# brucechin/OctopusZK

Hardware: AMD Instinct MI355X
Metric: BN254 G1 VariableBaseMSM Mscalar-mul/s at 2^20 (higher is better)
Workload: dtype u32; 1 GPU; VariableBaseMSM BN254 G1 2^20 random scalars/bases per GPU, bit-exact vs the serial CPU path (BASELINE.json configs[1]); n_per_gpu=1048576, window_bits=16, windows=8, glv=True, prepared_bases=False, msms_in_flight=3, schedule=pipeline3, parallelism=index-range shard x1, RCCL all-gather of 192-B partials + HIP point sum

## Files before the change

### octopuszk_amd/csrc/knobs.h

```cpp
#pragma once
#include <stdlib.h>
#include <string.h>

#include <atomic>
#include <mutex>

namespace ozk {

constexpr int KNOB_COMPUTED = -0x7fffffff;
constexpr int KNOB_STRING = KNOB_COMPUTED + 1;

#define OZK_KNOBS(X)                                                                                                     \
                                                   \
  X(MSM_GLV, "OZK_MSM_GLV", 1, "0: plain 256-bit windows instead of the GLV split (var MSM up to 2^23 pairs, fixed base)") \
  X(MSM_SIGNED, "OZK_MSM_SIGNED", 1, "0: unsigned window digits in the GLV form")                                        \
  X(MSM_C, "OZK_MSM_C", KNOB_COMPUTED, "window bits, 1..16 (default: the cost model's choice)")                          \
  X(MSM_L1, "OZK_MSM_L1", KNOB_COMPUTED, "sorted entries per level-1 lane (default: from the bucket size; 0 as unset)")   \
  X(MSM_L1_WHOLE, "OZK_MSM_L1_WHOLE", 1, "G1 level 1 by whole buckets on lane groups: 0 never, 1 on every plan that can take it (unset: where it pays)") \
  X(MSM_L1_ROUNDS, "OZK_MSM_L1_ROUNDS", 2, "most rounds of resident workgroups level 1 is rounded up to; 0: no rounding") \
  X(MSM_TAIL_MODE, "OZK_MSM_TAIL_MODE", -1, "0 / 1: force the latency / throughput shape of the window sums")            \
  X(MSM_TAIL_RC, "OZK_MSM_TAIL_RC", -1, "1: G1 throughput window sums by bucket rows and columns wherever the buffers take them (0 / unset: the serial levels)") \
  X(MSM_SMALL_SORT, "OZK_MSM_SMALL_SORT", 1, "0: small MSMs take the two-level sort too")                                \
  X(MSM_S_LAT, "OZK_MSM_S_LAT", KNOB_COMPUTED, "buckets per lane in a latency tail's fused first level (default: 8 G1, 4 G2)") \
  X(MSM_FIN_MAX, "OZK_MSM_FIN_MAX", 4, "elements per window left to the final one-wave kernel, 1..16")                   \
                                                                                                    \
  X(HOST_SLICES, "OZK_HOST_SLICES", 8, "most slices a host-buffer MSM is cut into; 1: no slicing")                       \
  X(HOST_SLICE_MIN_LOG, "OZK_HOST_SLICE_MIN_LOG", 18, "log2 of the smallest slice")                                      \
  X(SHARD, "OZK_SHARD", 0, "1: the JNI entries shard large calls over the visible devices")                              \
  X(SHARD_MIN_N, "OZK_SHARD_MIN_N", 1 << 21, "smallest call OZK_SHARD=1 shards")                                         \
  X(SHARD_COUNT, "OZK_SHARD_COUNT", 0, "shards of such a call; 0: one per device")                                       \
  X(SHARD_RCCL, "OZK_SHARD_RCCL", 1, "0: the partials of a sharded call go through the host, not RCCL")                  \
  X(COPY_HELPERS, "OZK_COPY_HELPERS", 3, "threads staging host buffers beside the caller, 0..11 (first use only)")       \
  X(HOST_TRACE, "OZK_HOST_TRACE", 0, "1: per-call host timings on stderr; 2: with absolute timestamps")                  \
                                                                                     \
  X(FB_WS, "OZK_FB_WS", KNOB_COMPUTED, "window bits of a GLV fixed-base table (default: cost model, at most the caller's)") \
  X(FB_AFFINE, "OZK_FB_AFFINE", 1, "0: Jacobian gather-add instead of affine table records")                             \
  X(FB_TABLE_CACHE, "OZK_FB_TABLE_CACHE", 1, "0: window tables are built per call")                                      \
  X(FB_TABLE_CACHE_MB, "OZK_FB_TABLE_CACHE_MB", 1024, "MiB of cached window tables per device")                          \
  X(FB_TABLE_CACHE_SECOND_USE, "OZK_FB_TABLE_CACHE_SECOND_USE", 1, "0: a table is cached on its first use")              \
  X(FB_HOST_RANGES, "OZK_FB_HOST_RANGES", 4, "ranges a host fixed-base call downloads its results in")                   \
  X(MM_WS, "OZK_MM_WS", KNOB_COMPUTED, "window bits of the shared-base batched MSM (default: from n)")                   \
                                                                                             \
  X(FFT_MAXK, "OZK_FFT_MAXK", 8, "most butterfly stages per pass, 3..10")                                                \
  X(FFT_PLAN, "OZK_FFT_PLAN", 1, "0: stages spread evenly over the passes")                                              \
  X(FFT_KS, "OZK_FFT_KS", KNOB_STRING, "explicit stages per pass, e.g. \"8,6,8\" (must sum to log2 n)")                  \
  X(FFT_TW_PYRAMID, "OZK_FFT_TW_PYRAMID", 1, "0: twiddles from the flat table")                                          \
  X(FFT_PLAN_CACHE, "OZK_FFT_PLAN_CACHE", 1, "0: twiddle tables are built per call")                                     \
  X(FFT_PLAN_CACHE_MB, "OZK_FFT_PLAN_CACHE_MB", 4096, "MiB of cached twiddle tables per device")                         \
  X(QAP_FOLD_SCALE, "OZK_QAP_FOLD_SCALE", 1, "0: the witness map scales in a pass of its own")                           \
  X(BACE_LDS_SLOTS, "OZK_BACE_LDS_SLOTS", 16, "circuit slots kept in LDS, 0..28")

enum Knob {
#define X(id, env, dflt, doc) K_##id,
  OZK_KNOBS(X)
#undef X
  K_COUNT
};
struct KnobInfo {
  const char* env;
  int dflt;
  const char* doc;
};
inline constexpr KnobInfo KNOBS[K_COUNT] = {
#define X(id, env, dflt, doc) {env, dflt, doc},
    OZK_KNOBS(X)
#undef X
};

struct KnobSnapshot {
  bool has[K_COUNT];
  int val[K_COUNT];
// ... 39 lines not shown
```

### octopuszk_amd/csrc/l1_whole.h

```cpp
#pragma once
#include <stdint.h>

#if !defined(OZK_HD)
#if defined(__HIPCC__)
#include <hip/hip_runtime.h>
#define OZK_HD __host__ __device__ __forceinline__
#else
#define OZK_HD inline
#endif
#endif

namespace ozk {

constexpr int WHOLE_G = 2;
constexpr int WHOLE_LANE_MAX = 255;
constexpr int WHOLE_NB_MAX = 128;

struct WholeGeom {
  int W;
  int NH;
  int nb;
  int g_top;
};
OZK_HD int whole_nbins(const WholeGeom& g) { return g.W * g.NH; }
constexpr uint32_t WHOLE_NO_ITEM = 0xffffffffu;
OZK_HD int whole_pad4(int x) { return (x + 3) & ~3; }
OZK_HD int whole_lanes_per_rank(const WholeGeom& g) {
  return whole_pad4(WHOLE_G * g.NH * (g.W - 1)) + whole_pad4(g.g_top * g.NH);
}
OZK_HD long long whole_lanes(const WholeGeom& g) { return (long long)g.nb * whole_lanes_per_rank(g); }
OZK_HD int whole_group(const WholeGeom& g, int bin) { return bin / g.NH == g.W - 1 ? g.g_top : WHOLE_G; }
OZK_HD uint32_t whole_limit(int G) { return (uint32_t)(G * WHOLE_LANE_MAX); }

OZK_HD uint32_t whole_rank(const uint32_t* cnt, int nb, int i) {
  const uint32_t c = cnt[i];
  uint32_t r = 0;
  for (int j = 0; j < nb; j++) r += (cnt[j] > c) || (cnt[j] == c && j < i);
  return r;
}
OZK_HD uint32_t whole_item_index(uint32_t rank, uint32_t bin, uint32_t nbins) { return rank * nbins + bin; }

OZK_HD void whole_lane_map(const WholeGeom& geo, uint32_t t, uint32_t* item, uint32_t* g, uint32_t* G) {
  const uint32_t per_rank = (uint32_t)whole_lanes_per_rank(geo);
  const uint32_t rank = t / per_rank, q = t - rank * per_rank;
  const uint32_t ordinary = (uint32_t)(WHOLE_G * geo.NH * (geo.W - 1));
  const uint32_t ordinary_pad = (uint32_t)whole_pad4((int)ordinary);
  uint32_t bin;
  bool pad;
  if (q < ordinary_pad) {
    bin = q / WHOLE_G;
    *g = q % WHOLE_G;
    *G = WHOLE_G;
    pad = q >= ordinary;
  } else {
    const uint32_t q2 = q - ordinary_pad;
    bin = (uint32_t)(geo.NH * (geo.W - 1)) + q2 / (uint32_t)geo.g_top;
    *g = q2 % (uint32_t)geo.g_top;
    *G = (uint32_t)geo.g_top;
    pad = q2 >= (uint32_t)(geo.g_top * geo.NH);
  }
  *item = pad ? WHOLE_NO_ITEM : whole_item_index(rank, bin, (uint32_t)whole_nbins(geo));
}

OZK_HD void whole_part(uint32_t count, uint32_t g, uint32_t G, uint32_t* first, uint32_t* len) {
  const uint32_t a = (count * g + G - 1) / G, b = (count * (g + 1) + G - 1) / G;
  *first = a;
  *len = b - a;
}

}
```

### octopuszk_amd/csrc/msm_var.cuh

```cuda
#pragma once
#include "curve.cuh"
#include "glv.cuh"
#include "l1_whole.h"
#include "wsum_rc.h"

namespace ozk {

constexpr u32 BID_NONE = 0xffffffffu;

struct MsmPlan {
  int n_in;
  int glv;
  int n;
  int sd;
  int c;
  int cb;
  int W;
  int L1;
  int LK;
  int S;
  int lone;
  int small_sort;
  int S_lat;
  int fin_max;
  int tail_mode;
  int tail_rc;
  int l1_whole;
  int l1_gtop;
};

OZK_HD u32 scalar_digit(const u32 (&s)[8], int w, int c) {
  const int bit = w * c;
  const int wi = bit >> 5, sh = bit & 31;
  u32 v = s[wi] >> sh;
  if (sh + c > 32 && wi + 1 < 8) v |= s[wi + 1] << (32 - sh);
  return v & ((1u << c) - 1u);
}

OZK_HD bool digit_decode(u32 code, int sd, u32& b, u32& neg) {
  if (sd) {
    const u32 t = code - 1u;
    b = t >> 1;
    neg = t & 1u;
  } else {
    b = code;
    neg = 0;
  }
  return code != 0;
}
template <class Emit>
OZK_HD void signed_digit_codes(const u32 (&e)[8], int c, int W, bool neg, Emit emit) {
  const u32 half = 1u << (c - 1);
  const u32 thr = (c == 16 && neg) ? half - 1u : half;
  u32 cy = 0;
  for (int w = 0; w < W; w++) {
    const u32 d = scalar_digit(e, w, c) + cy;
    cy = d > thr;
    const u32 m = cy ? (1u << c) - d : d;
    emit(w, (uint16_t)(m ? (((m - 1u) << 1) | (cy ^ (u32)neg)) + 1u : 0u));
  }
}

constexpr u32 SIDX_NEG = 0x80000000u;

#if defined(__HIPCC__)


template <class CV>
__global__ void __launch_bounds__(256) k_convert_bases(const u32* __restrict__ wire,
                                                       u32* __restrict__ aff, int n, int glv,
                                                       const uint8_t* __restrict__ neg_flags) {
  using IO = CurveIO<CV>;
  using EA = typename CV::EA;
  using ET = ElemTraits<EA>;
  const int i = blockIdx.x * blockDim.x + threadIdx.x;
  if (i >= n) return;
  const u32* p = wire + (size_t)i * IO::WIRE_JAC_WORDS;
  u32* o = aff + (size_t)i * IO::AFF_WORDS;
  Aff<EA> q;
  if (ET::wire_is_zero(p + 2 * IO::CW)) {
    q.x = EA(el_zero(q.x));
// ... 1004 lines not shown
          for (int q = s + 1; q <= e; q += 2) acc = xyzz_add(acc, IO::load_xyzz(pts + (size_t)q * IO::REC_WORDS));
          IO::store_rec_xyzz(acc, buckets + (size_t)bx * IO::REC_WORDS);
        } else if (e > s) {
          const u32 j = atomicAdd(&item_cnt[0], 1u);
          item_s[0][j] = (u32)s;
          item_span[0][j] = (uint8_t)(e - s);
        } else {
          IO::store_rec_xyzz(IO::load_xyzz(pts + (size_t)s * IO::REC_WORDS), buckets + (size_t)bx * IO::REC_WORDS);
        }
      }
    }
    bid_out[x] = out;
    alive += (out != BID_NONE);
  }
  if (t == 0 && n_slots > 0) {
    bid_out[0] = bid_in[0];
    alive += (bid_in[0] != BID_NONE);
  }
  for (int o = 32; o > 0; o >>= 1) alive += __shfl_xor(alive, o);
  if ((threadIdx.x & 63) == 0 && alive) atomicAdd(remaining, alive);
#pragma unroll 1
  for (int r = 0; LIST && r < ROUNDS; r++) {
    block_sync();
    const u32 len = (u32)__builtin_amdgcn_readfirstlane((int)item_cnt[r]);
    if (len == 0) break;
    const int cur = r & 1;
#pragma unroll 1
    for (u32 i = threadIdx.x; i < len; i += RUNMERGE_BLOCK) {
      const u32 s = item_s[cur][i];
      const u32 span = item_span[cur][i];
      u32* bucket = buckets + (size_t)bid_in[s] * IO::REC_WORDS;
      const u32 off = 2u * (u32)r + 1u;
      const u32* sum = r == 0 ? pts + (size_t)s * IO::REC_WORDS : bucket;
      const Xyzz<CV> acc = xyzz_add(IO::load_xyzz(sum), IO::load_xyzz(pts + ((size_t)s + off) * IO::REC_WORDS));
      IO::store_rec_xyzz(acc, bucket);
      if (off + 2u <= span) {
        const u32 j = atomicAdd(&item_cnt[r + 1], 1u);
        item_s[cur ^ 1][j] = s;
        item_span[cur ^ 1][j] = (uint8_t)span;
      }
    }
  }
}

constexpr int ITEMS_BLOCK = WHOLE_NB_MAX;
__device__ __forceinline__ u32 items_block_sum(u32 v, u32* wsum) {
#pragma unroll
  for (int o = 32; o > 0; o >>= 1) v += __shfl_xor(v, o);
  if ((threadIdx.x & 63) == 0) wsum[threadIdx.x >> 6] = v;
  block_sync();
  return wsum[0] + wsum[1];
}
static __global__ void __launch_bounds__(ITEMS_BLOCK)
k_bin_sums(const u32* __restrict__ hist, WholeGeom geo, int cb, int lo_bits, u32* __restrict__ binsum) {
  static_assert(ITEMS_BLOCK == 128, "two waves");
  __shared__ u32 wsum[2];
  const int t = threadIdx.x, bin = blockIdx.x;
  const int w = bin / geo.NH, h = bin - w * geo.NH;
  const u32 bucket0 = ((u32)w << cb) | ((u32)h << lo_bits);
  const u32 sum = items_block_sum(t < geo.nb ? hist[bucket0 + t] : 0u, wsum);
  if (t == 0) binsum[bin] = sum;
}
static __global__ void __launch_bounds__(ITEMS_BLOCK)
k_bucket_items(const u32* __restrict__ hist, const u32* __restrict__ binsum, WholeGeom geo, int cb, int lo_bits,
               u32 big_thresh, uint4* __restrict__ items, u32* __restrict__ bad) {
  __shared__ u32 cnt[WHOLE_NB_MAX];
  __shared__ u32 wsum[2];
  const int t = threadIdx.x, bin = blockIdx.x;
  const int w = bin / geo.NH, h = bin - w * geo.NH;
  const u32 bucket0 = ((u32)w << cb) | ((u32)h << lo_bits);
  const u32 c = t < geo.nb ? hist[bucket0 + t] : 0u;
  cnt[t] = c;
  u32 before = 0;
  for (int j = t; j < bin; j += ITEMS_BLOCK) before += binsum[j];
  const u32 base = items_block_sum(before, wsum);
  if (t >= geo.nb) return;
  u32 excl = 0, sum = 0;
  for (int j = 0; j < geo.nb; j++) {
    const u32 cj = cnt[j];
    sum += cj;
    excl += j < t ? cj : 0u;
  }
  const u32 rank = whole_rank(cnt, geo.nb, t);
  items[whole_item_index(rank, (u32)bin, (u32)whole_nbins(geo))] = make_uint4(base + excl, c, bucket0 + (u32)t, 0u);
  if (c > whole_limit(whole_group(geo, bin)) || sum > big_thresh) *bad = 1u;
}

template <int CTRL, class CV>
__device__ __forceinline__ Xyzz<CV> xyzz_quad_swap(const Xyzz<CV>& a) {
  using IO = CurveIO<CV>;
  constexpr int RW = IO::RW;
  u32 w[4 * RW];
  ElemTraits<typename CV::XX>::store_raw(a.X, w);
  ElemTraits<typename CV::XY>::store_raw(a.Y, w + RW);
  ElemTraits<typename CV::XZZ>::store_raw(a.ZZ, w + 2 * RW);
  ElemTraits<typename CV::XZZZ>::store_raw(a.ZZZ, w + 3 * RW);
#pragma unroll
  for (int k = 0; k < 4 * RW; k++) w[k] = (u32)__builtin_amdgcn_update_dpp(0, (int)w[k], CTRL, 0xf, 0xf, true);
  Xyzz<CV> b;
  b.X = ElemTraits<typename CV::XX>::load_raw(w);
  b.Y = ElemTraits<typename CV::XY>::load_raw(w + RW);
  b.ZZ = ElemTraits<typename CV::XZZ>::load_raw(w + 2 * RW);
  b.ZZZ = ElemTraits<typename CV::XZZZ>::load_raw(w + 3 * RW);
  return b;
}

template <class CV>
__global__ void __launch_bounds__(256)
k_l1_whole(const uint4* __restrict__ items, const uint2* __restrict__ sent, const u32* __restrict__ pts_in,
           const u32* __restrict__ bad, WholeGeom geo, u32 n_lanes, u32* __restrict__ buckets,
           unsigned long long* __restrict__ clk) {
  using IO = CurveIO<CV>;
  using Acc = RunAcc<CV, true>;
  if (*bad != 0u) return;
  unsigned long long w0 = 0, c0 = 0;
  if (clk != nullptr && threadIdx.x == 0) {
    w0 = (unsigned long long)wall_clock64();
    c0 = (unsigned long long)clock64();
    atomicMax(&clk[0], ~w0);
  }
  const u32 t = blockIdx.x * blockDim.x + threadIdx.x;
  u32 item, g, G;
  whole_lane_map(geo, t < n_lanes ? t : 0u, &item, &g, &G);
  const bool valid = t < n_lanes && item != WHOLE_NO_ITEM;
  uint4 it = items[valid ? item : 0u];
  if (!valid) it.y = 0u;
  u32 first, n_e;
  whole_part(it.y, g, G, &first, &n_e);
  Xyzz<CV> a = xyzz_from_affine<CV>(IO::aff_infinity());
  if (n_e != 0u) {
    const u32* idx_c = reinterpret_cast<const u32*>(sent + (size_t)it.x + first);
    u32 v_cur = idx_c[0];
    u32 v_next = idx_c[n_e > 1u ? 2 : 0];
    const __amdgpu_buffer_rsrc_t table = Acc::table_rsrc(pts_in);
    typename Acc::Raw r = Acc::load_raw_buf(table, v_cur);
    bool negate;
    auto take = [&](u32 k) {
      negate = (v_cur & SIDX_NEG) != 0;
      const auto q = Acc::decode_unsigned(r);
      const u32 k2 = (k + 2 < n_e) ? k + 2 : n_e - 1;
      r = Acc::load_raw_buf(table, v_next);
      v_cur = v_next;
      v_next = idx_c[2 * (size_t)k2];
      return q;
    };
    {
      const auto q = take(0u);
      a = xyzz_from_affine_signed<CV>(q, negate);
    }
    if (n_e > 1u) {
      const auto q = take(1u);
      a = xyzz_add_affine2_lazy(a, q, negate);
    }
    for (u32 k = 2; k < n_e; k++) {
      const auto q = take(k);
      a = xyzz_madd_lazy(a, q, negate);
    }
  }
  if (__ballot(G > 1u) != 0ull) {
    const Xyzz<CV> b = xyzz_quad_swap<0xB1, CV>(a);
    if (G > 1u) a = xyzz_add(a, b);
  }
  if (__ballot(G > 2u) != 0ull) {
    const Xyzz<CV> b = xyzz_quad_swap<0x4E, CV>(a);
    if (G > 2u) a = xyzz_add(a, b);
  }
  if (g == 0u && it.y != 0u) IO::store_rec_xyzz(a, buckets + (size_t)it.z * IO::REC_WORDS);
  if (clk != nullptr && (threadIdx.x & 63) == 0) {
    const unsigned long long w1 = (unsigned long long)wall_clock64();
    atomicMax(&clk[1], w1);
    if (threadIdx.x == 0) {
      atomicAdd(&clk[2], (unsigned long long)clock64() - c0);
      atomicAdd(&clk[3], w1 - w0);
    }
  }
}

template <class CV, bool FIRSTLEVEL>
__global__ void __launch_bounds__(256)
k_wsum(const u32* __restrict__ A_in, const u32* __restrict__ R_in, const u32* __restrict__ hist,
       int m_in, int S, int g, u32* __restrict__ A_out, u32* __restrict__ R_out, int m_out, int W, int prio) {
  using IO = CurveIO<CV>;
  if (prio) __builtin_amdgcn_s_setprio(3);
  const int t = blockIdx.x * blockDim.x + threadIdx.x;
  if (t >= m_out * W) return;
  const int w = t / m_out, j = t - w * m_out;
  const size_t base = (size_t)w * m_in;
  const int lo = j * S;
  int hi = lo + S;
  if (hi > m_in) hi = m_in;
  Jac<CV> run = jac_infinity<CV>(), ws = jac_infinity<CV>(), asum = jac_infinity<CV>();
  for (int e = hi - 1; e >= lo; e--) {
    if constexpr (FIRSTLEVEL) {
      if (hist[base + e] != 0) run = jac_add(run, IO::load_rec(R_in + (base + e) * IO::REC_WORDS));
    } else {
      run = jac_add(run, IO::load_jac(R_in + (base + e) * IO::JAC_WORDS));
    }
    if (e > lo) ws = jac_add(ws, run);
    if constexpr (!FIRSTLEVEL) asum = jac_add(asum, IO::load_jac(A_in + (base + e) * IO::JAC_WORDS));
  }
  for (int k = 0; k < g; k++) ws = jac_dbl(ws);
  if constexpr (!FIRSTLEVEL) ws = jac_add(ws, asum);
  IO::store_jac(ws, A_out + ((size_t)w * m_out + j) * IO::JAC_WORDS);
  IO::store_jac(run, R_out + ((size_t)w * m_out + j) * IO::JAC_WORDS);
}

template <class CV>
__device__ __forceinline__ Jac<CV> shfl_down_jac(const Jac<CV>& p, int o) {
  Jac<CV> r;
  r.X = shfl_down_el(p.X, o);
  r.Y = shfl_down_el(p.Y, o);
  r.Z = shfl_down_el(p.Z, o);
  return r;
}

template <class CV>
__device__ __forceinline__ void wave_combine(Jac<CV>& A, Jac<CV>& T, int l, int valid, int g) {
  for (int o = 1; o < valid; o <<= 1) {
    const Jac<CV> t = shfl_down_jac(T, o);
    const Jac<CV> s = jac_add(T, t);
    if (l + o < 64) T = s;
  }
  Jac<CV> U = T;
  for (int k = 0; k < g; k++) U = jac_dbl(U);
  const Jac<CV> AV = jac_add(A, U);
  Jac<CV> V = (l >= 1) ? AV : A;
  int top = 1;
  while (top < valid) top <<= 1;
// ... 317 lines not shown
```

### octopuszk_amd/csrc/msm_var_driver.cuh

```cuda
#pragma once
#include <hip/hip_ext.h>
#include <pthread.h>
#include <stdlib.h>

#include <atomic>
#include <vector>

#include "msm_var.cuh"
#include "host_ctx.h"
#include "fq2.cuh"

namespace ozk {

enum { PROF_OFF = 0, PROF_EVENTS = 1, PROF_CLOCK = 2 };
struct ProfState {
  pthread_mutex_t mu = PTHREAD_MUTEX_INITIALIZER;
  std::atomic<int> mode{PROF_OFF};
  int src = PROF_EVENTS;
  int every = 1, seen = 0;
  int count = 0;
  std::vector<hipEvent_t> e0, e1;
  bool created = false;
  int ev_device = -1;
  unsigned long long* d_clk = nullptr;
// ... 57 lines not shown
    if (p.glv) {
      const int top_bits = 127 - (Wk - 1) * k;
      const long long per_top = top_bits >= 1 ? ((long long)p.n >> (top_bits - sd_ok > 0 ? top_bits - sd_ok : 0)) : (long long)p.n;
      long long l1 = ((long long)p.n >> (k - sd_ok)) * 5 / 16;
      if (l1 < 40) l1 = 40;
      if (per_top / l1 > 10) cost += 4.0e6;
    }
    if (cost < best) {
      best = cost;
      c = k;
    }
  }
  c = knob_or(K_MSM_C, c);
  if (c < 1) c = 1;
  if (c > 16) c = 16;
  p.c = c;
  p.sd = sd_ok && c >= 2;
  p.cb = c - p.sd;
  p.W = ((p.glv ? 128 : 256) + c - 1) / c;
  {
    const long long per_bucket = (long long)p.n >> p.cb;
    long long l1 = per_bucket * 5 / 16;
    long long l1_min = p.n >= (1 << 20) ? 52 : 40;
    if (p.glv) {
      const long long cap = (long long)p.n * p.W;
      long long fit = cap / 65536;
      const int top_bits = 127 - (p.W - 1) * p.c;
      const int tb = top_bits - p.sd;
      const long long per_top = (top_bits >= 1 && top_bits < p.c) ? ((long long)p.n >> (tb > 0 ? tb : 0)) : per_bucket;
      const long long pieces = (per_top + 9) / 10;
      if (fit < pieces) fit = pieces;
      if (fit < 8) fit = 8;
      if (fit < l1_min) l1_min = fit;
    }
    if (l1 < l1_min) l1 = l1_min;
    if (l1 > 1024) l1 = 1024;
    p.L1 = knob_or(K_MSM_L1, (int)l1);
  }
  if (p.L1 < 2) p.L1 = 2;
  p.LK = PLAN_LK;
  p.S = PLAN_S;
  p.lone = 0;
  p.small_sort = p.n <= SORTS_MAX_N && p.cb <= SORTS_MAX_CB && knob(K_MSM_SMALL_SORT) != 0;
  p.S_lat = p.S;
  p.fin_max = knob(K_MSM_FIN_MAX);
  if (p.fin_max < 1) p.fin_max = 1;
  if (p.fin_max > 16) p.fin_max = 16;
  p.tail_mode = knob(K_MSM_TAIL_MODE);
  if (p.tail_mode != 0 && p.tail_mode != 1) p.tail_mode = -1;
  p.tail_rc = knob(K_MSM_TAIL_RC);
  if (p.tail_rc != 1) p.tail_rc = 0;
  p.l1_whole = 0;
  p.l1_gtop = WHOLE_G;
  return p;
}

template <class CV>
static MsmPlan plan_for(int n, bool lone) {
  MsmPlan p = make_plan(n);
  p.lone = lone;
  const long long max_rounds = knob(K_MSM_L1_ROUNDS);
  bool rounded = false;
  if ((CV::LDS_ACC || lone) && knob_or(K_MSM_L1, 0) == 0 && max_rounds != 0) {
    static int cu_count = 0;
    if (cu_count == 0) {
      int dev = 0, cus = 0;
      if (hipGetDevice(&dev) == hipSuccess && hipDeviceGetAttribute(&cus, hipDeviceAttributeMultiprocessorCount, dev) == hipSuccess &&
          cus > 0)
        cu_count = cus;
      else
        cu_count = 256;
    }
    const int slots = (CV::LDS_ACC ? 2 : 3) * cu_count;
    const long long cap = (long long)p.n * p.W;
    const long long blocks = ((cap + p.L1 - 1) / p.L1 + 255) / 256;
    long long rounds = blocks / slots > 0 ? blocks / slots : 1;
    if (rounds > max_rounds) rounds = max_rounds;
    long long l1 = (cap + 256LL * slots * rounds - 1) / (256LL * slots * rounds);
    if (l1 > p.L1 && l1 <= 1024) {
      p.L1 = (int)l1;
      rounded = true;
    }
  }
  const int s_lat = knob_or(K_MSM_S_LAT, std::is_same<CV, G1Cfg>::value && p.cb >= 13 ? 8 : p.S);
  if (s_lat >= 2 && s_lat <= 64) p.S_lat = 1 << ilog2((uint32_t)s_lat);
  const int whole_knob = knob_or(K_MSM_L1_WHOLE, -1);
  bool whole_pays = true;
  if (lone) {
    const int tb = 127 - (p.W - 1) * p.c;
    const long long per_bucket = (long long)p.n >> p.cb;
    const long long per_top = (tb >= 1 && tb < p.c) ? ((long long)p.n >> (tb - p.sd > 0 ? tb - p.sd : 0)) : per_bucket;
    whole_pays = !rounded && per_bucket / WHOLE_G <= p.L1 && per_top / 4 <= p.L1;
  }
  if (std::is_same<CV, G1Cfg>::value && p.glv && p.sd && !p.small_sort && (whole_knob == -1 ? whole_pays : whole_knob != 0)) {
    const int top_bits = 127 - (p.W - 1) * p.c;
    p.l1_whole = 1;
    p.l1_gtop = (top_bits >= 1 && top_bits < p.c) ? 4 : WHOLE_G;
  }
  return p;
}

struct L1PathLast {
  int planned = -1;
  const u32* d_bad = nullptr;
};
inline thread_local L1PathLast g_l1_path_last;
// ... 157 lines not shown
  }
  if (p.small_sort) {
    hipLaunchKernelGGL(k_sort_small, dim3(p.W), dim3(SORTS_BLOCK), 0, st, L.digits, n, p.cb, p.sd, L.total, L.hist, L.sent);
    if (order_ev) OZK_HIP(hipStreamWaitEvent(st, order_ev, 0));
    OZK_HIP(hipGetLastError());
    return OZK_OK;
  }
  const size_t lds1 = (size_t)L.NH * sizeof(u32);
  hipLaunchKernelGGL(k_sort1_count, dim3(L.nblk, p.W), dim3(SORT_BLOCK), lds1, st, L.digits, n, L.lo_bits, p.sd,
                     L.NH, L.nblk, L.C1);
  const int items = SCAN_BLOCK * SCAN_ITEMS;
  const int nb = (int)((L.nC1 + items - 1) / items);
  hipLaunchKernelGGL(k_scan_blocksum, dim3(nb), dim3(SCAN_BLOCK), 0, st, L.C1, (int)L.nC1, L.blocksum);
  hipLaunchKernelGGL(k_scan_top, dim3(1), dim3(1024), 0, st, L.blocksum, nb, L.total);
  hipLaunchKernelGGL(k_scan_final, dim3(nb), dim3(SCAN_BLOCK), 0, st, L.C1, (int)L.nC1, L.blocksum, L.P1);
  const size_t lds_sc = ((size_t)2 * L.NH + 2 * SORT_CHUNK) * sizeof(u32);
  hipLaunchKernelGGL(k_sort1_scatter, dim3(L.nblk, p.W), dim3(SORT_BLOCK), lds_sc, st, L.digits, n, L.lo_bits,
                     p.sd, L.NH, L.nblk, L.P1, L.total, L.nC1, L.coarse);
  const int nbins = p.W * L.NH;
  const u32 sign_bit = p.sd ? 0x80u : 0u;
  const u32 big_thresh = (u32)(n / 64) > SORT_BIG ? (u32)(n / 64) : SORT_BIG;
  if (L.cap / ((size_t)big_thresh + 1) > (size_t)SORTBIG_MAXBINS)
    return fail(OZK_E_INVALID, "window plan c=%d (W=%d) at n=%d can produce more than %d oversized sort bins",
                p.c, p.W, p.n_in, SORTBIG_MAXBINS);
  hipLaunchKernelGGL(k_sort2, dim3(nbins), dim3(SORT2_BLOCK), 0, st, L.coarse, L.P1, L.total, p.cb, L.lo_bits, L.NH,
                     sign_bit, L.nblk, nbins, big_thresh, L.hist, L.sent);
  if (order_ev) OZK_HIP(hipStreamWaitEvent(st, order_ev, 0));
  hipLaunchKernelGGL(k_sortbig_list, dim3(1), dim3(256), 0, st, L.P1, L.total, L.nblk, nbins, big_thresh, L.bigbins);
  hipLaunchKernelGGL(k_sortbig_count, dim3(1024), dim3(SORT_BLOCK), 0, st, L.coarse, L.bigbins,
                     (1u << L.lo_bits) - 1u, L.bigT);
  hipLaunchKernelGGL(k_sortbig_scan, dim3(SORTBIG_MAXBINS), dim3(256), 0, st, L.bigbins, L.bigT, p.cb, L.lo_bits, L.NH,
                     L.hist);
  hipLaunchKernelGGL(k_sortbig_scatter, dim3(1024), dim3(SORT_BLOCK), 0, st, L.coarse, L.bigbins, L.bigT, p.cb,
                     L.lo_bits, sign_bit, L.NH, L.sent);
  OZK_HIP(hipGetLastError());
  return OZK_OK;
}

enum { ACCUM_ALL = 0, ACCUM_LEVEL1 = 1, ACCUM_REST = 2 };
template <class CV>
int var_msm_accum(const MsmPlan& p, void* sorted, size_t sorted_bytes, void* accum_ws, size_t accum_ws_bytes,
                         void* tail, size_t tail_bytes, hipStream_t st, const void* prepared = nullptr,
                         int part = ACCUM_ALL) {
  hip_clear_stale();
  using CT = CV;
  RegionBytes rb;
  MsmLayout L = make_layout3<CV>(p, sorted, nullptr, accum_ws, &rb, prepared);
  if (rb.sorted > sorted_bytes || rb.accum_ws > accum_ws_bytes)
    return fail(OZK_E_INVALID, "accumulate buffers too small: need %zu + %zu bytes, got %zu + %zu", rb.sorted,
                rb.accum_ws, sorted_bytes, accum_ws_bytes);
  const size_t tneed = tail_layout<CV>(p, L, tail, tail_bytes);
  if (tneed > tail_bytes) return fail(OZK_E_INVALID, "tail buffer too small: need %zu bytes, got %zu", tneed, tail_bytes);
  const int TB = 256;
  const bool whole = !CV::LDS_ACC && p.l1_whole && (1 << L.lo_bits) <= WHOLE_NB_MAX &&
                     L.NB * sizeof(uint4) + (size_t)p.W * L.NH * sizeof(u32) <= rb.accum_ws;
  u32* whole_bad = L.total + 2;
  g_l1_path_last.planned = whole ? 1 : 0;
  g_l1_path_last.d_bad = whole_bad;
  size_t lanes = (L.cap + p.L1 - 1) / p.L1;
  if (part != ACCUM_REST) {
  hipEvent_t prof_e0 = nullptr, prof_e1 = nullptr;
  unsigned long long* clk = nullptr;
  g_prof.claim(&prof_e0, &prof_e1, &clk);
  const bool prof = prof_e0 != nullptr;
  size_t acc_lds = CV::LDS_ACC ? (size_t)RunAccLds<CV>::LDS_WORDS * TB * sizeof(u32) : 0;
  if (!CV::LDS_ACC) acc_lds = L1_LDS_G1;
  auto launch_l1 = [&](auto kern) {
    if (acc_lds > 65536)
      OZK_HIP(hipFuncSetAttribute((const void*)kern, hipFuncAttributeMaxDynamicSharedMemorySize, (int)acc_lds));
    hipExtLaunchKernelGGL(kern, dim3((unsigned)((lanes + TB - 1) / TB)), dim3(TB), (uint32_t)acc_lds, st,
                          prof && !whole ? prof_e0 : (hipEvent_t) nullptr, prof && !whole ? prof_e1 : (hipEvent_t) nullptr, 0u,
                          (const u32*)nullptr, (const u32*)L.sent, (const u32*)L.aff, (const u32*)L.total, 0, p.L1,
                          L.buckets, L.slot_bid[0], L.slot_pts[0], (int)lanes, clk, whole ? (const u32*)whole_bad : (const u32*)nullptr);
    return OZK_OK;
  };
  if constexpr (!CV::LDS_ACC) {
    if (whole) {
      const WholeGeom geo{p.W, L.NH, 1 << L.lo_bits, p.l1_gtop};
      const u32 big_thresh = (u32)(p.n / 64) > SORT_BIG ? (u32)(p.n / 64) : SORT_BIG;
      uint4* items = (uint4*)accum_ws;
      u32* binsum = (u32*)(items + L.NB);
      hipLaunchKernelGGL(k_bin_sums, dim3((unsigned)whole_nbins(geo)), dim3(ITEMS_BLOCK), 0, st, (const u32*)L.hist, geo,
                         p.cb, L.lo_bits, binsum);
      hipLaunchKernelGGL(k_bucket_items, dim3((unsigned)whole_nbins(geo)), dim3(ITEMS_BLOCK), 0, st, (const u32*)L.hist,
                         (const u32*)binsum, geo, p.cb, L.lo_bits, big_thresh, items, whole_bad);
      const long long wl = whole_lanes(geo);
      hipExtLaunchKernelGGL((k_l1_whole<CV>), dim3((unsigned)((wl + TB - 1) / TB)), dim3(TB), (uint32_t)acc_lds, st,
                            prof ? prof_e0 : (hipEvent_t) nullptr, prof ? prof_e1 : (hipEvent_t) nullptr, 0u,
                            (const uint4*)items, (const uint2*)L.sent, (const u32*)L.aff, (const u32*)whole_bad, geo,
                            (u32)wl, L.buckets, clk);
    }
  }
  if (int rc_l1 = launch_l1(k_segreduce<CV, true, CV::LAZY_MADD>)) return rc_l1;
  }
  if (part == ACCUM_LEVEL1) {
    OZK_HIP(hipGetLastError());
    return OZK_OK;
  }
  size_t n_in = 2 * lanes;
  static_assert(RUNMERGE_BLOCK == 256, "k_runmerge's work list is sized for this launch");
  hipLaunchKernelGGL((k_runmerge<CT>), dim3((unsigned)((lanes + TB - 1) / TB)), dim3(TB), 0, st, L.slot_bid[0],
                     L.slot_pts[0], (int)n_in, L.buckets, L.slot_bid2, L.total + 1, (const u32*)L.hist, L.hist_t, L.NB,
                     whole ? (const u32*)whole_bad : (const u32*)nullptr);
  int cur = 0;
  bool first_generic = true;
  while (true) {
    lanes = (n_in + p.LK - 1) / p.LK;
    if (!first_generic && (int)lanes <= SMALL_LEVEL_LANES) {
      hipLaunchKernelGGL((k_segreduce_small<CT>), dim3(1), dim3(TB), 0, st, L.total + 1, (int)n_in, p.LK, L.buckets,
                         L.slot_bid[cur], L.slot_pts[cur], L.slot_bid[cur ^ 1], L.slot_pts[cur ^ 1]);
      break;
    }
    hipLaunchKernelGGL((k_segreduce<CT, false>), dim3((unsigned)((lanes + TB - 1) / TB)), dim3(TB), 0, st,
                       first_generic ? L.slot_bid2 : L.slot_bid[cur], (const u32*)nullptr, L.slot_pts[cur],
                       L.total + 1, (int)n_in, p.LK, L.buckets, L.slot_bid[cur ^ 1], L.slot_pts[cur ^ 1], (int)lanes,
                       (unsigned long long*)nullptr);
    first_generic = false;
    if (lanes == 1) break;
    n_in = 2 * lanes;
    cur ^= 1;
  }
  OZK_HIP(hipGetLastError());
  return OZK_OK;
}

template <class CV>
int var_msm_head(const MsmPlan& p, const void* d_bases, const void* d_scalars, void* ws, size_t ws_bytes, void* tail,
                        size_t tail_bytes, hipStream_t st, hipEvent_t order_ev = nullptr,
                        const void* prepared = nullptr) {
  const RegionBytes rb = region_bytes<CV>(p);
  if (rb.sorted + rb.sort_ws + rb.accum_ws > ws_bytes)
    return fail(OZK_E_INVALID, "workspace too small: need %zu bytes, got %zu", rb.sorted + rb.sort_ws + rb.accum_ws,
                ws_bytes);
  uint8_t* w = (uint8_t*)ws;
  int rc = var_msm_sort<CV>(p, d_bases, d_scalars, w, rb.sorted, w + rb.sorted, rb.sort_ws, st, order_ev, prepared);
  if (rc) return rc;
  return var_msm_accum<CV>(p, w, rb.sorted, w + rb.sorted + rb.sort_ws, rb.accum_ws, tail, tail_bytes, st, prepared);
}

inline thread_local int g_tail_form_last = -1;
template <class CV>
bool tail_rc_applies(const MsmPlan& p, const MsmLayout& L) {
  using IO = CurveIO<CV>;
// ... 353 lines not shown
```

Measured before the change: 745.2 Mscalar-mul/s.

## Order whole-bucket level-1 items by part length and merge lane groups densely via LDS

The whole-bucket level-1 item list can now be ordered globally by per-lane part length, using a key-class histogram table built in the bin-sum kernel and slots claimed atomically in the item kernel. Blocks from the two lane-group regions are interleaved, so each wave gets lanes with similar loop trip counts and less divergence. Full blocks also merge lane-group partners by writing points to LDS and having half the threads read pairs, instead of quad permutes that keep every lane live. The cost is an extra memset, atomics and key-class scans in the prep kernels, and LDS traffic with a block barrier during the merge.

```diff
diff --git a/octopuszk_amd/csrc/knobs.h b/octopuszk_amd/csrc/knobs.h
--- a/octopuszk_amd/csrc/knobs.h
+++ b/octopuszk_amd/csrc/knobs.h
@@ -17,6 +17,8 @@
   X(MSM_C, "OZK_MSM_C", KNOB_COMPUTED, "window bits, 1..16 (default: the cost model's choice)")                          \
   X(MSM_L1, "OZK_MSM_L1", KNOB_COMPUTED, "sorted entries per level-1 lane (default: from the bucket size; 0 as unset)")   \
   X(MSM_L1_WHOLE, "OZK_MSM_L1_WHOLE", 1, "G1 level 1 by whole buckets on lane groups: 0 never, 1 on every plan that can take it (unset: where it pays)") \
+  X(MSM_L1_ORDER, "OZK_MSM_L1_ORDER", 1, "item order of the whole-bucket level 1: 0 by rank inside the sort bin, 1 by part length over the whole MSM") \
+  X(MSM_L1_DENSE, "OZK_MSM_L1_DENSE", 1, "0: every workgroup of the whole-bucket level 1 merges lane groups by quad permutes, none densely through LDS") \
   X(MSM_L1_ROUNDS, "OZK_MSM_L1_ROUNDS", 2, "most rounds of resident workgroups level 1 is rounded up to; 0: no rounding") \
   X(MSM_TAIL_MODE, "OZK_MSM_TAIL_MODE", -1, "0 / 1: force the latency / throughput shape of the window sums")            \
   X(MSM_TAIL_RC, "OZK_MSM_TAIL_RC", -1, "1: G1 throughput window sums by bucket rows and columns wherever the buffers take them (0 / unset: the serial levels)") \
diff --git a/octopuszk_amd/csrc/l1_whole.h b/octopuszk_amd/csrc/l1_whole.h
--- a/octopuszk_amd/csrc/l1_whole.h
+++ b/octopuszk_amd/csrc/l1_whole.h
@@ -68,4 +68,67 @@
   *len = b - a;
 }
 
+constexpr int WHOLE_KEYS = 128;
+constexpr int WHOLE_WAVE = 64, WHOLE_TB = 256;
+constexpr int WHOLE_TABLE_WORDS = 2 * 2 * WHOLE_KEYS;
+OZK_HD uint32_t whole_key(uint32_t count, uint32_t G) {
+  const uint32_t k = (count + G - 1) / G;
+  return k < (uint32_t)(WHOLE_KEYS - 1) ? k : (uint32_t)(WHOLE_KEYS - 1);
 }
+OZK_HD int whole_regions(const WholeGeom& g) { return g.g_top == WHOLE_G ? 1 : 2; }
+OZK_HD int whole_bin_region(const WholeGeom& g, int bin) { return (whole_regions(g) == 2 && bin / g.NH == g.W - 1) ? 1 : 0; }
+OZK_HD uint32_t whole_region_group(const WholeGeom& g, int r) { return r == 0 ? (uint32_t)WHOLE_G : (uint32_t)g.g_top; }
+OZK_HD uint32_t whole_region_items(const WholeGeom& g, int r) {
+  const uint32_t top = (uint32_t)(g.NH * g.nb), all = (uint32_t)(g.W * g.NH * g.nb);
+  if (whole_regions(g) == 1) return r == 0 ? all : 0u;
+  return r == 0 ? all - top : top;
+}
+OZK_HD uint32_t whole_region_lanes(const WholeGeom& g, int r) {
+  const uint32_t l = whole_region_group(g, r) * whole_region_items(g, r);
+  return (l + (uint32_t)(WHOLE_WAVE - 1)) & ~(uint32_t)(WHOLE_WAVE - 1);
+}
+OZK_HD long long whole_lanes_len(const WholeGeom& g) { return (long long)whole_region_lanes(g, 0) + whole_region_lanes(g, 1); }
+OZK_HD uint32_t whole_class_base(const uint32_t* T, uint32_t key) {
+  uint32_t s = 0;
+  for (uint32_t k = (uint32_t)WHOLE_KEYS - 1; k > key; k--) s += T[k];
+  return s;
+}
+OZK_HD void whole_class_bases(const uint32_t* T, uint32_t* base) {
+  for (uint32_t k = 0; k < (uint32_t)WHOLE_KEYS; k++) base[k] = whole_class_base(T, k);
+}
+OZK_HD void whole_len_blocks(const WholeGeom& g, uint32_t* nb0, uint32_t* nb1) {
+  const uint32_t all = (uint32_t)((whole_lanes_len(g) + WHOLE_TB - 1) / WHOLE_TB);
+  *nb0 = whole_region_lanes(g, 0) / (uint32_t)WHOLE_TB;
+  *nb1 = all - *nb0;
+}
+OZK_HD uint32_t whole_block_interleave(uint32_t p, uint32_t nb0, uint32_t nb1) {
+  const unsigned long long n = (unsigned long long)nb0 + nb1;
+  const uint32_t before = (uint32_t)((unsigned long long)p * nb1 / n), upto = (uint32_t)(((unsigned long long)p + 1) * nb1 / n);
+  return upto > before ? nb0 + before : p - before;
+}
+OZK_HD void whole_lane_map_len(const WholeGeom& geo, uint32_t u, uint32_t* item, uint32_t* g, uint32_t* G) {
+  const uint32_t l0 = whole_region_lanes(geo, 0), n0 = whole_region_items(geo, 0);
+  if (u < l0) {
+    *G = (uint32_t)WHOLE_G;
+    *g = u % (uint32_t)WHOLE_G;
+    const uint32_t i = u / (uint32_t)WHOLE_G;
+    *item = i < n0 ? i : WHOLE_NO_ITEM;
+  } else {
+    const uint32_t q = u - l0, gt = (uint32_t)geo.g_top;
+    *G = gt;
+    *g = q % gt;
+    const uint32_t i = q / gt;
+    *item = i < whole_region_items(geo, 1) ? n0 + i : WHOLE_NO_ITEM;
+  }
+}
+
+OZK_HD bool whole_block_dense(const WholeGeom& geo, int order, uint32_t block, uint32_t n_lanes) {
+  const unsigned long long t0 = (unsigned long long)block * WHOLE_TB;
+  if (t0 + WHOLE_TB > n_lanes) return false;
+  if (order == 1) return t0 + WHOLE_TB <= whole_region_lanes(geo, 0);
+  const uint32_t per_rank = (uint32_t)whole_lanes_per_rank(geo);
+  const uint32_t q0 = (uint32_t)(t0 % per_rank);
+  return q0 + (uint32_t)WHOLE_TB <= (uint32_t)whole_pad4(WHOLE_G * geo.NH * (geo.W - 1));
+}
+
+}
diff --git a/octopuszk_amd/csrc/msm_var.cuh b/octopuszk_amd/csrc/msm_var.cuh
--- a/octopuszk_amd/csrc/msm_var.cuh
+++ b/octopuszk_amd/csrc/msm_var.cuh
@@ -27,6 +27,8 @@
   int tail_rc;
   int l1_whole;
   int l1_gtop;
+  int l1_order;
+  int l1_dense;
 };
 
 OZK_HD u32 scalar_digit(const u32 (&s)[8], int w, int c) {
@@ -1137,38 +1139,79 @@
   return wsum[0] + wsum[1];
 }
 static __global__ void __launch_bounds__(ITEMS_BLOCK)
-k_bin_sums(const u32* __restrict__ hist, WholeGeom geo, int cb, int lo_bits, u32* __restrict__ binsum) {
-  static_assert(ITEMS_BLOCK == 128, "two waves");
+k_bin_sums(const u32* __restrict__ hist, WholeGeom geo, int cb, int lo_bits, u32* __restrict__ binsum, int order,
+           u32* __restrict__ table) {
+  static_assert(ITEMS_BLOCK == 128 && WHOLE_KEYS == ITEMS_BLOCK, "two waves; one thread per key class");
   __shared__ u32 wsum[2];
-  const int t = threadIdx.x, bin = blockIdx.x;
-  const int w = bin / geo.NH, h = bin - w * geo.NH;
-  const u32 bucket0 = ((u32)w << cb) | ((u32)h << lo_bits);
-  const u32 sum = items_block_sum(t < geo.nb ? hist[bucket0 + t] : 0u, wsum);
-  if (t == 0) binsum[bin] = sum;
-}
-static __global__ void __launch_bounds__(ITEMS_BLOCK)
-k_bucket_items(const u32* __restrict__ hist, const u32* __restrict__ binsum, WholeGeom geo, int cb, int lo_bits,
-               u32 big_thresh, uint4* __restrict__ items, u32* __restrict__ bad) {
-  __shared__ u32 cnt[WHOLE_NB_MAX];
-  __shared__ u32 wsum[2];
+  __shared__ u32 keys[WHOLE_KEYS];
   const int t = threadIdx.x, bin = blockIdx.x;
   const int w = bin / geo.NH, h = bin - w * geo.NH;
   const u32 bucket0 = ((u32)w << cb) | ((u32)h << lo_bits);
   const u32 c = t < geo.nb ? hist[bucket0 + t] : 0u;
+  if (order == 1) {
+    keys[t] = 0u;
+    block_sync();
+    if (t < geo.nb) atomicAdd(&keys[whole_key(c, (u32)whole_group(geo, bin))], 1u);
+  }
+  const u32 sum = items_block_sum(c, wsum);
+  if (t == 0) binsum[bin] = sum;
+  if (order == 1) {
+    const u32 v = keys[t];
+    if (v != 0u) atomicAdd(&table[whole_bin_region(geo, bin) * WHOLE_KEYS + t], v);
+  }
+}
+static __global__ void __launch_bounds__(ITEMS_BLOCK)
+k_bucket_items(const u32* __restrict__ hist, const u32* __restrict__ binsum, WholeGeom geo, int cb, int lo_bits,
+               u32 big_thresh, uint4* __restrict__ items, u32* __restrict__ bad, int order, u32* __restrict__ table) {
+  __shared__ u32 cnt[WHOLE_NB_MAX];
+  __shared__ u32 wsum[2];
+  __shared__ u32 keyv[WHOLE_NB_MAX], cls[WHOLE_KEYS], slot0[WHOLE_KEYS];
+  const int t = threadIdx.x, bin = blockIdx.x;
+  const int w = bin / geo.NH, h = bin - w * geo.NH;
+  const u32 bucket0 = ((u32)w << cb) | ((u32)h << lo_bits);
+  const u32 c = t < geo.nb ? hist[bucket0 + t] : 0u;
+  const u32 G = (u32)whole_group(geo, bin);
+  const int region = whole_bin_region(geo, bin);
+  const u32 key = whole_key(c, G);
   cnt[t] = c;
+  if (order == 1) {
+    keyv[t] = key;
+    cls[t] = table[region * WHOLE_KEYS + t];
+  }
   u32 before = 0;
   for (int j = t; j < bin; j += ITEMS_BLOCK) before += binsum[j];
   const u32 base = items_block_sum(before, wsum);
-  if (t >= geo.nb) return;
+  const bool live = t < geo.nb;
   u32 excl = 0, sum = 0;
   for (int j = 0; j < geo.nb; j++) {
     const u32 cj = cnt[j];
     sum += cj;
     excl += j < t ? cj : 0u;
   }
-  const u32 rank = whole_rank(cnt, geo.nb, t);
-  items[whole_item_index(rank, (u32)bin, (u32)whole_nbins(geo))] = make_uint4(base + excl, c, bucket0 + (u32)t, 0u);
-  if (c > whole_limit(whole_group(geo, bin)) || sum > big_thresh) *bad = 1u;
+  const uint4 it = make_uint4(base + excl, c, bucket0 + (u32)t, G);
+  if (order != 1) {
+    if (!live) return;
+    const u32 rank = whole_rank(cnt, geo.nb, t);
+    items[whole_item_index(rank, (u32)bin, (u32)whole_nbins(geo))] = it;
+    if (c > whole_limit((int)G) || sum > big_thresh) *bad = 1u;
+    return;
+  }
+  u32 same = 0, same_before = 0;
+  for (int j = 0; j < geo.nb; j++) {
+    const bool e = keyv[j] == key;
+    same += e ? 1u : 0u;
+    same_before += (e && j < t) ? 1u : 0u;
+  }
+  const u32 cbase = whole_class_base(cls, key);
+  if (live && same_before == 0u) slot0[key] = atomicAdd(&table[(2 + region) * WHOLE_KEYS + key], same);
+  block_sync();
+  if (!live) return;
+  const u32 slot = cbase + slot0[key] + same_before;
+  if (slot < whole_region_items(geo, region))
+    items[(region == 1 ? whole_region_items(geo, 0) : 0u) + slot] = it;
+  else
+    *bad = 1u;
+  if (c > whole_limit((int)G) || sum > big_thresh) *bad = 1u;
 }
 
 template <int CTRL, class CV>
@@ -1194,9 +1237,12 @@
 __global__ void __launch_bounds__(256)
 k_l1_whole(const uint4* __restrict__ items, const uint2* __restrict__ sent, const u32* __restrict__ pts_in,
            const u32* __restrict__ bad, WholeGeom geo, u32 n_lanes, u32* __restrict__ buckets,
-           unsigned long long* __restrict__ clk) {
+           unsigned long long* __restrict__ clk, int order, int dense_on, u32 nb0, u32 nb1) {
   using IO = CurveIO<CV>;
   using Acc = RunAcc<CV, true>;
+  constexpr int RW = IO::RW;
+  static_assert(WHOLE_TB == 256, "the launch bound, the LDS layout");
+  static_assert(WHOLE_G >= 2, "the first merge step below is unconditional: every lane group has a partner lane");
   if (*bad != 0u) return;
   unsigned long long w0 = 0, c0 = 0;
   if (clk != nullptr && threadIdx.x == 0) {
@@ -1204,9 +1250,24 @@
     c0 = (unsigned long long)clock64();
     atomicMax(&clk[0], ~w0);
   }
-  const u32 t = blockIdx.x * blockDim.x + threadIdx.x;
+  auto stamp_end = [&]() {
+    if (clk != nullptr && (threadIdx.x & 63) == 0) {
+      const unsigned long long w1 = (unsigned long long)wall_clock64();
+      atomicMax(&clk[1], w1);
+      if (threadIdx.x == 0) {
+        atomicAdd(&clk[2], (unsigned long long)clock64() - c0);
+        atomicAdd(&clk[3], w1 - w0);
+      }
+    }
+  };
+  const u32 block = order == 1 ? whole_block_interleave(blockIdx.x, nb0, nb1) : blockIdx.x;
+  const bool dense = dense_on != 0 && whole_block_dense(geo, order, block, n_lanes);
+  const u32 t = block * blockDim.x + threadIdx.x;
   u32 item, g, G;
-  whole_lane_map(geo, t < n_lanes ? t : 0u, &item, &g, &G);
+  if (order == 1)
+    whole_lane_map_len(geo, t < n_lanes ? t : 0u, &item, &g, &G);
+  else
+    whole_lane_map(geo, t < n_lanes ? t : 0u, &item, &g, &G);
   const bool valid = t < n_lanes && item != WHOLE_NO_ITEM;
   uint4 it = items[valid ? item : 0u];
   if (!valid) it.y = 0u;
@@ -1242,23 +1303,54 @@
       a = xyzz_madd_lazy(a, q, negate);
     }
   }
-  if (__ballot(G > 1u) != 0ull) {
-    const Xyzz<CV> b = xyzz_quad_swap<0xB1, CV>(a);
-    if (G > 1u) a = xyzz_add(a, b);
-  }
-  if (__ballot(G > 2u) != 0ull) {
-    const Xyzz<CV> b = xyzz_quad_swap<0x4E, CV>(a);
+  extern __shared__ __attribute__((aligned(16))) u32 ozk_whole_lds[];
+  if (dense) {
+    {
+      u32 w[4 * RW];
+      ElemTraits<typename CV::XX>::store_raw(a.X, w);
+      ElemTraits<typename CV::XY>::store_raw(a.Y, w + RW);
+      ElemTraits<typename CV::XZZ>::store_raw(a.ZZ, w + 2 * RW);
+      ElemTraits<typename CV::XZZZ>::store_raw(a.ZZZ, w + 3 * RW);
+#pragma unroll
+      for (int k = 0; k < 4 * RW; k++) ozk_whole_lds[k * WHOLE_TB + threadIdx.x] = w[k];
+      if (g == 0u) ozk_whole_lds[4 * RW * WHOLE_TB + (threadIdx.x >> 1)] = it.y != 0u ? it.z : WHOLE_NO_ITEM;
+    }
+    block_sync();
+    if (threadIdx.x >= WHOLE_TB / 2) {
+      stamp_end();
+      return;
+    }
+  }
+  Xyzz<CV> b;
+  u32 store_id;
+  if (dense) {
+    u32 wa[4 * RW], wb[4 * RW];
+#pragma unroll
+    for (int k = 0; k < 4 * RW; k++) {
+      const uint2 p = reinterpret_cast<const uint2*>(ozk_whole_lds + k * WHOLE_TB)[threadIdx.x];
+      wa[k] = p.x;
+      wb[k] = p.y;
+    }
+    a.X = ElemTraits<typename CV::XX>::load_raw(wa);
+    a.Y = ElemTraits<typename CV::XY>::load_raw(wa + RW);
+    a.ZZ = ElemTraits<typename CV::XZZ>::load_raw(wa + 2 * RW);
+    a.ZZZ = ElemTraits<typename CV::XZZZ>::load_raw(wa + 3 * RW);
+    b.X = ElemTraits<typename CV::XX>::load_raw(wb);
+    b.Y = ElemTraits<typename CV::XY>::load_raw(wb + RW);
+    b.ZZ = ElemTraits<typename CV::XZZ>::load_raw(wb + 2 * RW);
+    b.ZZZ = ElemTraits<typename CV::XZZZ>::load_raw(wb + 3 * RW);
+    store_id = ozk_whole_lds[4 * RW * WHOLE_TB + threadIdx.x];
+  } else {
+    b = xyzz_quad_swap<0xB1, CV>(a);
+    store_id = (g == 0u && it.y != 0u) ? it.z : WHOLE_NO_ITEM;
+  }
+  a = xyzz_add(a, b);
+  if (!dense && __ballot(G > 2u) != 0ull) {
+    b = xyzz_quad_swap<0x4E, CV>(a);
     if (G > 2u) a = xyzz_add(a, b);
   }
-  if (g == 0u && it.y != 0u) IO::store_rec_xyzz(a, buckets + (size_t)it.z * IO::REC_WORDS);
-  if (clk != nullptr && (threadIdx.x & 63) == 0) {
-    const unsigned long long w1 = (unsigned long long)wall_clock64();
-    atomicMax(&clk[1], w1);
-    if (threadIdx.x == 0) {
-      atomicAdd(&clk[2], (unsigned long long)clock64() - c0);
-      atomicAdd(&clk[3], w1 - w0);
-    }
-  }
+  if (store_id != WHOLE_NO_ITEM) IO::store_rec_xyzz(a, buckets + (size_t)store_id * IO::REC_WORDS);
+  stamp_end();
 }
 
 template <class CV, bool FIRSTLEVEL>
diff --git a/octopuszk_amd/csrc/msm_var_driver.cuh b/octopuszk_amd/csrc/msm_var_driver.cuh
--- a/octopuszk_amd/csrc/msm_var_driver.cuh
+++ b/octopuszk_amd/csrc/msm_var_driver.cuh
@@ -133,6 +133,8 @@
   if (p.tail_rc != 1) p.tail_rc = 0;
   p.l1_whole = 0;
   p.l1_gtop = WHOLE_G;
+  p.l1_order = knob(K_MSM_L1_ORDER) != 0 ? 1 : 0;
+  p.l1_dense = knob(K_MSM_L1_DENSE) != 0 ? 1 : 0;
   return p;
 }
 
@@ -396,8 +398,9 @@
   const size_t tneed = tail_layout<CV>(p, L, tail, tail_bytes);
   if (tneed > tail_bytes) return fail(OZK_E_INVALID, "tail buffer too small: need %zu bytes, got %zu", tneed, tail_bytes);
   const int TB = 256;
+  const size_t whole_table_words = p.l1_order == 1 ? (size_t)WHOLE_TABLE_WORDS : 0;
   const bool whole = !CV::LDS_ACC && p.l1_whole && (1 << L.lo_bits) <= WHOLE_NB_MAX &&
-                     L.NB * sizeof(uint4) + (size_t)p.W * L.NH * sizeof(u32) <= rb.accum_ws;
+                     L.NB * sizeof(uint4) + ((size_t)p.W * L.NH + whole_table_words) * sizeof(u32) <= rb.accum_ws;
   u32* whole_bad = L.total + 2;
   g_l1_path_last.planned = whole ? 1 : 0;
   g_l1_path_last.d_bad = whole_bad;
@@ -423,16 +426,22 @@
       const WholeGeom geo{p.W, L.NH, 1 << L.lo_bits, p.l1_gtop};
       const u32 big_thresh = (u32)(p.n / 64) > SORT_BIG ? (u32)(p.n / 64) : SORT_BIG;
       uint4* items = (uint4*)accum_ws;
-      u32* binsum = (u32*)(items + L.NB);
+      u32* table = (u32*)(items + L.NB);
+      u32* binsum = table + whole_table_words;
+      static_assert(TB == WHOLE_TB && ((size_t)4 * CurveIO<CV>::RW * WHOLE_TB + WHOLE_TB / 2) * sizeof(u32) <= (size_t)L1_LDS_G1,
+                    "the dense merge's LDS lies inside what the launch asks for anyway");
+      if (p.l1_order == 1) OZK_HIP(hipMemsetAsync(table, 0, WHOLE_TABLE_WORDS * sizeof(u32), st));
       hipLaunchKernelGGL(k_bin_sums, dim3((unsigned)whole_nbins(geo)), dim3(ITEMS_BLOCK), 0, st, (const u32*)L.hist, geo,
-                         p.cb, L.lo_bits, binsum);
+                         p.cb, L.lo_bits, binsum, p.l1_order, table);
       hipLaunchKernelGGL(k_bucket_items, dim3((unsigned)whole_nbins(geo)), dim3(ITEMS_BLOCK), 0, st, (const u32*)L.hist,
-                         (const u32*)binsum, geo, p.cb, L.lo_bits, big_thresh, items, whole_bad);
-      const long long wl = whole_lanes(geo);
+                         (const u32*)binsum, geo, p.cb, L.lo_bits, big_thresh, items, whole_bad, p.l1_order, table);
+      const long long wl = p.l1_order == 1 ? whole_lanes_len(geo) : whole_lanes(geo);
+      u32 nb0 = 0, nb1 = 0;
+      whole_len_blocks(geo, &nb0, &nb1);
       hipExtLaunchKernelGGL((k_l1_whole<CV>), dim3((unsigned)((wl + TB - 1) / TB)), dim3(TB), (uint32_t)acc_lds, st,
                             prof ? prof_e0 : (hipEvent_t) nullptr, prof ? prof_e1 : (hipEvent_t) nullptr, 0u,
                             (const uint4*)items, (const uint2*)L.sent, (const u32*)L.aff, (const u32*)whole_bad, geo,
-                            (u32)wl, L.buckets, clk);
+                            (u32)wl, L.buckets, clk, p.l1_order, p.l1_dense, nb0, nb1);
     }
   }
   if (int rc_l1 = launch_l1(k_segreduce<CV, true, CV::LAZY_MADD>)) return rc_l1;
```

Result: faster. 762.8 Mscalar-mul/s, median of 6 (+2.4%).
